# mikeferguson/ndt_2d

Hardware: AMD Instinct MI355X
Metric: pose-candidates x beams scored per second (higher is better)
Workload: dtype f64

## Files before the change

### ndt_2d_amd/csrc/ndt2d_device_fn.h

```cpp
#ifndef NDT2D_DEVICE_FN_H_
#define NDT2D_DEVICE_FN_H_

#include <hip/hip_runtime.h>
#include <math.h>

#include "ndt2d_kernels.h"

namespace ndt2d
{

constexpr int kWave = 64;
constexpr int kRecord = 12;
constexpr double kNoIndex = 1.0e308;
constexpr double kPadCoord = -1.0e300;

template <bool POW2>
__device__ __forceinline__ uint32_t cell_index(const GridDesc & g, double px, double py)
{
  const double tx = px - g.origin_x;
  const double ty = py - g.origin_y;
  double fx, fy;
  if (POW2)
  {
    fx = tx * g.inv_cell_size;
    fy = ty * g.inv_cell_size;
  }
  else
  {
    fx = tx / g.cell_size;
    fy = ty / g.cell_size;
  }
  const bool inside = (tx >= 0.0) & (ty >= 0.0) & (fx < static_cast<double>(g.size_x)) &
                      (fy < static_cast<double>(g.size_y));
  const uint32_t gx = static_cast<uint32_t>(fx);
  const uint32_t gy = static_cast<uint32_t>(fy);
  return inside ? gy * g.size_x + gx : g.ncell;
}

__device__ __forceinline__ double record_exponent(double mx, double my, double h00,
                                                  double h01, double h11, double px, double py)
{
  const double q0 = px - mx;
  const double q1 = py - my;
  const double r0 = q0 * h00 + q1 * h01;
  const double r1 = q0 * h01 + q1 * h11;
  return r0 * q0 + r1 * q1;
}

__device__ __forceinline__ double record_likelihood(double mx, double my, double h00,
                                                    double h01, double h11, double px,
                                                    double py)
{
  return exp(record_exponent(mx, my, h00, h01, h11, px, py));
}

__device__ __forceinline__ double fma3(double a, double b, double c)
{
  double d;
  asm("v_fma_f64 %0, %1, %2, %3" : "=v"(d) : "v"(a), "v"(b), "v"(c));
  return d;
}
#ifndef NDT2D_EXP_SCALAR_CONSTANTS
#define NDT2D_EXP_SCALAR_CONSTANTS 0
#endif
template <uint32_t HI, uint32_t LO>
__device__ __forceinline__ double fma3k(double a, double b)
{
  double d;
#if NDT2D_EXP_SCALAR_CONSTANTS
  uint32_t lo, hi;
  asm volatile("s_mov_b32 %0, %2\n\ts_mov_b32 %1, %3" : "=s"(lo), "=s"(hi) : "n"(LO), "n"(HI));
  const double c = __hiloint2double(static_cast<int>(hi), static_cast<int>(lo));
  asm("v_fma_f64 %0, %1, %2, %3" : "=v"(d) : "v"(a), "v"(b), "s"(c));
#else
  asm("v_fma_f64 %0, %1, %2, %3" : "=v"(d) : "v"(a), "v"(b), "v"(__hiloint2double(static_cast<int>(HI), static_cast<int>(LO))));
#endif
  return d;
}

__device__ __forceinline__ double exp_of_exponent(double x)
{
  asm("v_max_f64 %0, %1, %2" : "=v"(x) : "v"(x), "s"(-1000.0));
  const double n = rint(x * 1.4426950408889634);
  double r = fma(n, -0.6931471805599453, x);
  r = fma(n, -2.3190468138462996e-17, r);
  double p = fma3k<0x3e928af3u, 0xfca7ab0cu>(r, 0x1.ade156a5dcb37p-26);
  p = fma3k<0x3ec71deeu, 0x623fde64u>(r, p);
  p = fma3k<0x3efa0199u, 0x7c89e6b0u>(r, p);
  p = fma3k<0x3f2a01a0u, 0x14761f6eu>(r, p);
  p = fma3k<0x3f56c16cu, 0x1852b7b0u>(r, p);
  p = fma3k<0x3f811111u, 0x11122322u>(r, p);
  p = fma3k<0x3fa55555u, 0x555502a1u>(r, p);
  p = fma3k<0x3fc55555u, 0x55555511u>(r, p);
  p = fma3k<0x3fe00000u, 0x0000000bu>(r, p);
  asm("v_fma_f64 %0, %1, %2, 1.0" : "=v"(p) : "v"(r), "v"(p));
  asm("v_fma_f64 %0, %1, %2, 1.0" : "=v"(p) : "v"(r), "v"(p));
  return ldexp(p, static_cast<int>(n));
}

__device__ __forceinline__ bool wave_any(bool p)
{
  return __builtin_amdgcn_ballot_w64(p) != 0ull;
}

constexpr double kExpOverflowAbove = 0x1.62e42fefa39efp+9;

__device__ __forceinline__ double exp_score(double e)
{
  double r = exp_of_exponent(e);
  if (__builtin_expect(wave_any(!(e <= kExpOverflowAbove)), 0))
  {
    r = (e != e) ? e + e : (e > kExpOverflowAbove ? HUGE_VAL : r);
  }
  return r;
}

__device__ __forceinline__ double negligible_below(double s)
{
  const double from_sum =
    fma(static_cast<double>(__builtin_amdgcn_frexp_exp(s) - 1), 0.6931471805599453, -38.0);
  return (s > 0.0 && from_sum > -746.0) ? from_sum : -746.0;
}

template <bool LDS_GRID>
__device__ __forceinline__ double indexed_exponent(const GridDesc & g, const double * lds_cells,
                                                   uint32_t idx, double px, double py)
{
  double2 a, b, c;
  if (LDS_GRID)
  {
    const double2 * rec = reinterpret_cast<const double2 *>(lds_cells + idx * kCellDoubles);
    a = rec[0];
    b = rec[1];
    c = rec[2];
  }
  else
  {
    const double2 * rec =
      reinterpret_cast<const double2 *>(g.cells_global + static_cast<size_t>(idx) * kCellStrideGlobal);
    a = rec[0];
    b = rec[1];
    c = rec[2];
  }
  return record_exponent(a.x, a.y, b.x, b.y, c.x, px, py);
}

template <bool LDS_GRID>
__device__ __forceinline__ double indexed_likelihood(const GridDesc & g, const double * lds_cells,
                                                     uint32_t idx, double px, double py)
{
  return exp(indexed_exponent<LDS_GRID>(g, lds_cells, idx, px, py));
}

template <bool LDS_GRID, bool POW2>
__device__ __forceinline__ double point_likelihood(const GridDesc & g, const double * lds_cells,
                                                   double px, double py)
{
  return indexed_likelihood<LDS_GRID>(g, lds_cells, cell_index<POW2>(g, px, py), px, py);
}

__device__ __forceinline__ void stage_grid_to_lds(const GridDesc & g, double * lds_cells)
{
  const uint32_t n2 = (g.ncell + 1) * kCellDoubles / 2;
  const double2 * src = reinterpret_cast<const double2 *>(g.cells_lds_image);
  double2 * dst = reinterpret_cast<double2 *>(lds_cells);
  for (uint32_t i = threadIdx.x; i < n2; i += blockDim.x)
  {
    dst[i] = src[i];
  }
}

__device__ __forceinline__ double wave_sum(double v)
{
#pragma unroll
  for (int off = kWave / 2; off > 0; off >>= 1)
  {
    v += __shfl_xor(v, off, kWave);
  }
  return v;
}

constexpr int kDppQuadXor1 = 0xb1;
constexpr int kDppQuadXor2 = 0x4e;
constexpr int kDppRowHalfMirror = 0x141;
constexpr int kDppRowMirror = 0x140;
constexpr int kDppRowBcast15 = 0x142;
constexpr int kDppRowBcast31 = 0x143;

template <int CTRL, int ROW_MASK>
__device__ __forceinline__ double dpp_f64(double v, double fallback)
{
  const int lo = __builtin_amdgcn_update_dpp(__double2loint(fallback), __double2loint(v), CTRL,
                                             ROW_MASK, 0xf, false);
  const int hi = __builtin_amdgcn_update_dpp(__double2hiint(fallback), __double2hiint(v), CTRL,
                                             ROW_MASK, 0xf, false);
  return __hiloint2double(hi, lo);
}

__device__ __forceinline__ double wave_sum_to_last_lane(double v)
{
  v += dpp_f64<kDppQuadXor1, 0xf>(v, 0.0);
  v += dpp_f64<kDppQuadXor2, 0xf>(v, 0.0);
  v += dpp_f64<kDppRowHalfMirror, 0xf>(v, 0.0);
  v += dpp_f64<kDppRowMirror, 0xf>(v, 0.0);
  v += dpp_f64<kDppRowBcast15, 0xa>(v, 0.0);
  v += dpp_f64<kDppRowBcast31, 0xc>(v, 0.0);
  return v;
}

__device__ __forceinline__ double shortest_angular_distance(double from, double to)
{
  const double kPi = 3.14159265358979323846;
  const double r = fmod((to - from) + kPi, 2.0 * kPi);
  return r <= 0.0 ? r + kPi : r - kPi;
}

__device__ __forceinline__ void store_host(double * p, double v)
{
  __hip_atomic_store(p, v, __ATOMIC_RELAXED, __HIP_MEMORY_SCOPE_SYSTEM);
}
__device__ __forceinline__ void raise_host_flag(double * flag_slot, unsigned long long seq)
{
  asm volatile("s_waitcnt vmcnt(0)" ::: "memory");
  __hip_atomic_store(reinterpret_cast<unsigned long long *>(flag_slot), seq, __ATOMIC_RELAXED,
                     __HIP_MEMORY_SCOPE_SYSTEM);
}

#ifdef NDT2D_TEST_HOOKS
constexpr unsigned long long kDonePollTicks = 50ull * 1000 * 1000;
#else
constexpr unsigned long long kDonePollTicks = 1000ull * 1000 * 1000;
#endif
struct BoundedPoll
{
  uint32_t trips = 0;
  unsigned long long since = 0;
  __device__ __forceinline__ bool expired()
  {
    if ((++trips & 1023u) != 0u) return false;
    const unsigned long long now = wall_clock64();
    if (since == 0)
    {
      since = now | 1ull;
      return false;
    }
    return now - since > kDonePollTicks;
  }
};

#ifdef NDT2D_TEST_HOOKS
static __device__ int g_test_drop_done = 0;
#define NDT2D_TEST_DROPS_DONE(index) (g_test_drop_done != 0 && static_cast<uint32_t>(g_test_drop_done - 1) == static_cast<uint32_t>(index))
#else
#define NDT2D_TEST_DROPS_DONE(index) false
#endif

__device__ __forceinline__ bool better(double s_a, double i_a, double s_b, double i_b)
{
  return (s_a < s_b) | ((s_a == s_b) & (i_a < i_b));
}

constexpr int kNearTieLog2 = 36;

__device__ __forceinline__ void merge_best(double os, double oi, double & s, double & i)
{
  double larger;
  asm("v_max_f64 %0, |%1|, |%2|" : "=v"(larger) : "v"(os), "v"(s));
  const bool near = (ldexp(fabs(os - s), kNearTieLog2) <= larger) & (oi < kNoIndex) & (i < kNoIndex);
  if (better(os, oi, s, i))
  {
    s = os;
    i = oi;
  }
  if (near) i = floor(i) + 0.5;
}

template <int CTRL, int ROW_MASK>
__device__ __forceinline__ void best_step(double & s, double & i)
{
  const double os = dpp_f64<CTRL, ROW_MASK>(s, s);
  const double oi = dpp_f64<CTRL, ROW_MASK>(i, kNoIndex);
  merge_best(os, oi, s, i);
}

__device__ __forceinline__ void wave_best_to_last_lane(double & s, double & i)
{
  best_step<kDppQuadXor1, 0xf>(s, i);
  best_step<kDppQuadXor2, 0xf>(s, i);
  best_step<kDppRowHalfMirror, 0xf>(s, i);
  best_step<kDppRowMirror, 0xf>(s, i);
  best_step<kDppRowBcast15, 0xa>(s, i);
  best_step<kDppRowBcast31, 0xc>(s, i);
}

}

#endif
```

### ndt_2d_amd/csrc/ndt2d_match_lane.hip

```cpp
#include <cmath>
#include <cstdlib>

#include <type_traits>

#include "ndt2d_lane_fn.h"

namespace ndt2d
{

namespace
{

constexpr uint32_t kDynamicItemsFromBeams = 256;
constexpr int kLaneThreads = 1024;
constexpr int kLaneThreadsSmall = 256;
#ifndef NDT2D_LANE_THREADS_COMPACT
#define NDT2D_LANE_THREADS_COMPACT 768
#endif
constexpr int kLaneThreadsCompact = NDT2D_LANE_THREADS_COMPACT;
#define NDT2D_LANE_COMPACT_WAVES_PER_EU (NDT2D_LANE_THREADS_COMPACT / 128)

__global__ void __launch_bounds__(256) outer_table_kernel(const MatchArgs a, double4 * outer,
                                                          uint8_t * map_out, const LaneGeom geo)
{
  {
    const GridDesc & g = a.grid;
    const uint32_t n_map = static_cast<uint32_t>(kMapStride) * geo.map_h;
    for (uint32_t i = blockIdx.x * 256 + threadIdx.x; i < n_map; i += gridDim.x * 256)
    {
      const int32_t mx = static_cast<int32_t>(i & (kMapStride - 1));
      const int32_t my = static_cast<int32_t>(i >> 8);
      if (geo.block_log2 > 0)
      {
        const int32_t cells = 1 << geo.block_log2;
        map_out[i] = block_byte(g, mx * cells - geo.pad + geo.win_x0, my * cells - geo.pad + geo.win_y0, cells);
        continue;
      }
      const int32_t sub = 1 << geo.sub_log2;
      const int32_t cx = (mx >> geo.sub_log2) - geo.pad + geo.win_x0;
      const int32_t cy = (my >> geo.sub_log2) - geo.pad + geo.win_y0;
      map_out[i] = sub_cell_byte(g, cx, cy, mx & (sub - 1), my & (sub - 1), geo.sub_log2);
    }
  }

  if (blockIdx.x == 0 && threadIdx.x < kItemShards) a.next_item[threadIdx.x * kItemShardStride] = 0u;
  const uint64_t n = static_cast<uint64_t>(a.th_end - a.th_begin) * a.n_beams;
  for (uint64_t i = static_cast<uint64_t>(blockIdx.x) * 256 + threadIdx.x; i < n;
       i += static_cast<uint64_t>(gridDim.x) * 256)
  {
    const uint32_t t = static_cast<uint32_t>(i / a.n_beams);
    const uint32_t b = static_cast<uint32_t>(i - static_cast<uint64_t>(t) * a.n_beams);
    const uint32_t ith = a.th_begin + t * a.th_stride;
    const double ct = a.cos_th[ith];
    const double st = a.sin_th[ith];
    const double2 p = reinterpret_cast<const double2 *>(a.beams_xy)[b];
    double4 o;
    o.x = p.x * ct - p.y * st + a.pose_x;
    o.y = p.x * st + p.y * ct + a.pose_y;
    double kx = ((o.x - a.grid.origin_x) * a.grid.inv_cell_size + (geo.pad - geo.win_x0)) * geo.unit_scale;
    double ky = ((o.y - a.grid.origin_y) * a.grid.inv_cell_size + (geo.pad - geo.win_y0)) * geo.unit_scale;
    kx = !(kx >= geo.k_min) ? geo.k_min : (kx > geo.k_max_x ? geo.k_max_x : kx);
    ky = !(ky >= geo.k_min) ? geo.k_min : (ky > geo.k_max_y ? geo.k_max_y : ky);
    o.z = kTwo52 + (rint(ky) * kTwo24 + rint(kx)) + kNearBias;
    o.w = 0.0;
    outer[i] = o;
  }
}

__device__ __forceinline__ void item_step(uint32_t item, uint32_t patches, uint32_t th_mid, uint32_t & t,
                                          uint32_t & p)
{
  const uint32_t rank = item / patches;
  p = item - rank * patches;
  t = (rank & 1u) ? th_mid + (rank + 1u) / 2u : th_mid - rank / 2u;
}

__device__ __forceinline__ void item_place(uint32_t item, uint32_t patches, uint32_t patches_1d,
                                           uint32_t th_mid, uint32_t & t, uint32_t & pxi, uint32_t & pyi)
{
  uint32_t p;
  item_step(item, patches, th_mid, t, p);
  pxi = p / patches_1d;
  pyi = p - pxi * patches_1d;
}

__device__ __forceinline__ double packed_offset(double dx, double dy, double inv_scaled)
{
  return rint(dy * inv_scaled) * kTwo24 + rint(dx * inv_scaled);
}

__device__ __forceinline__ double no_index_here()
{
  static_assert(kNoIndex == 1.0e308, "the literal below is 1.0e308");
  uint32_t lo, hi;
  asm volatile("v_mov_b32 %0, 0x85ebc8a0\n\tv_mov_b32 %1, 0x7fe1ccf3" : "=v"(lo), "=v"(hi));
  return __hiloint2double(static_cast<int>(hi), static_cast<int>(lo));
}

template <int THREADS, bool POW2, bool LDS_RECORDS, bool DYNAMIC_ITEMS, bool COMPACT, bool PARTS = false,
          bool STRIPS = false>
__device__ __forceinline__ void match_lane_body(
  const MatchArgs & a, const double4 * __restrict__ outer, const uint8_t * __restrict__ map_image,
  const LaneGeom & geo)
{
  extern __shared__ __align__(16) double lds[];
  const GridDesc & g = a.grid;
#if defined(NDT2D_LANE_HIST) || defined(NDT2D_LANE_PATHS)
  if (blockIdx.x == 0 && threadIdx.x == 0) g_lane_hist = a.scores;
#endif
  uint8_t * lds_map = reinterpret_cast<uint8_t *>(lds);
  const uint32_t map_bytes = static_cast<uint32_t>(geo.map_h) * kMapStride;
  const uint32_t rank_bytes = COMPACT ? compact_rank_bytes(g.ncell) : 0u;
  double * lds_cells = lds + (map_bytes + rank_bytes) / sizeof(double);

  if (COMPACT)
  {
    const uint4 * src_rank = reinterpret_cast<const uint4 *>(g.cell_rank);
    uint4 * dst_rank = reinterpret_cast<uint4 *>(lds_map + map_bytes + kRankLead);
    for (uint32_t i = threadIdx.x; i < (rank_bytes - kRankLead) / 16; i += THREADS) dst_rank[i] = src_rank[i];
    if (threadIdx.x == 0)
    {
      reinterpret_cast<uint16_t *>(lds_map + map_bytes + kRankLead)[-1] = static_cast<uint16_t>(g.n_occ);
    }
    const uint32_t n2 = (g.n_occ + 1) * kCellDoubles / 2;
    const double2 * src = reinterpret_cast<const double2 *>(g.compact_records);
    double2 * dst = reinterpret_cast<double2 *>(lds_cells);
    for (uint32_t i = threadIdx.x; i < n2; i += THREADS) dst[i] = src[i];
  }
  else if (LDS_RECORDS)
  {
    stage_grid_to_lds(g, lds_cells);
  }
  {
    const uint32_t n16 = static_cast<uint32_t>(kMapStride) * geo.map_h / 16;
    const uint4 * src = reinterpret_cast<const uint4 *>(map_image);
    uint4 * dst = reinterpret_cast<uint4 *>(lds_map);
    for (uint32_t i = threadIdx.x; i < n16; i += THREADS) dst[i] = src[i];
  }
  __syncthreads();

#ifdef NDT2D_LANE_TRACE
  const unsigned long long trace_t0 = wall_clock64();
  unsigned long long trace_last = trace_t0, trace_max = 0, trace_last_start = trace_t0;
  uint32_t trace_items = 0, trace_prev_item = 0, trace_flagged = 0;
#endif
  LaneCtx c;
  c.rank_address = map_bytes + (COMPACT ? kRankLead : 0u);
  c.lds_cells_address = map_bytes + rank_bytes;
  c.sub_log2 = static_cast<uint32_t>(geo.sub_log2);
  c.exact_index = geo.block_log2 > 0 ? 1u : 0u;
  c.idx_bias = static_cast<uint32_t>(geo.pad - geo.win_y0) * g.size_x +
               static_cast<uint32_t>(geo.pad - geo.win_x0);
  c.size_x = g.size_x;

  const uint32_t lane = threadIdx.x & (kWave - 1);
  const uint32_t wave = __builtin_amdgcn_readfirstlane(threadIdx.x >> 6);
  const uint32_t n_lin = a.n_lin;
  static_assert(!STRIPS || (DYNAMIC_ITEMS && !PARTS), "strip tiles: the unsplit dynamic-item forms only");
  const LaneTiling tiling = lane_tiling(n_lin, STRIPS);
  const uint32_t patches = tiling.per_theta;
  const uint32_t n_items = (a.th_end - a.th_begin) * patches * (PARTS ? a.beam_parts : 1u);
  constexpr uint32_t kLaneWaves = THREADS / kWave;
  const uint32_t n_workers = gridDim.x * kLaneWaves;
  const uint32_t worker = wave * gridDim.x + blockIdx.x;
  const uint64_t per_theta = static_cast<uint64_t>(n_lin) * n_lin;
  const uint32_t th_mid = (a.th_end - a.th_begin - 1u) / 2u;
  const uint32_t home_shard = blockIdx.x % kItemShards;
  const double inv_scaled = geo.inv_scaled;

  double best_s = 0.0;
  double best_i = kNoIndex;
  double acc[10];
#pragma unroll
  for (int k = 0; k < 10; ++k) acc[k] = 0.0;
  for (uint32_t item = worker; item < n_items;)
  {
    uint32_t t, p;
#ifdef NDT2D_LANE_TRACE
    {
      const unsigned long long now = wall_clock64();
      if (trace_items > 0 && now - trace_last > trace_max) trace_max = now - trace_last;
      if (trace_items > 0 && a.scores != nullptr && lane == 0)
      {
        a.scores[5 * 8192 + 150000 + trace_prev_item] = static_cast<double>(now - trace_last);
        a.scores[5 * 8192 + 300000 + trace_prev_item] = static_cast<double>(trace_flagged);
      }
      trace_flagged = 0;
      trace_prev_item = item;
      trace_last = now;
      trace_last_start = now;
      ++trace_items;
      if (a.scores != nullptr && lane == 0) a.scores[5 * 8192 + item] = static_cast<double>(now);
    }
#endif
    const uint32_t whole_item = PARTS ? item / a.beam_parts : item;
    const uint32_t part = PARTS ? item - whole_item * a.beam_parts : 0u;
    item_step(whole_item, patches, th_mid, t, p);
    uint32_t x0, y0, h_log2, x_end;
    if (STRIPS)
    {
      lane_tile(tiling, n_lin, p, x0, y0, h_log2, x_end);
    }
    else
    {
      x0 = p / tiling.row * kPatch;
      y0 = (p - p / tiling.row * tiling.row) * kPatch;
      h_log2 = 3;
      x_end = n_lin;
    }
    const bool strip_tile = STRIPS && p >= tiling.core;
    uint32_t lane_here = lane;
    asm volatile("" : "+v"(lane_here));
    const uint32_t ix = x0 + (lane_here >> h_log2);
    const uint32_t iy = y0 + (lane_here & ((1u << h_log2) - 1u));
    const double dx = a.dlin[min(ix, x_end - 1)];
    const double dy = a.dlin[min(iy, n_lin - 1)];
    const double dxy = packed_offset(dx, dy, inv_scaled);
    const double4 * __restrict__ row = outer + static_cast<size_t>(t) * a.n_beams;

    double sum = 0.0;
    SkipState skip = skip_state(0.0, geo.no_skip);
    NDT2D_PATH(200, 1);
    const double dxy_corner = __hiloint2double(__builtin_amdgcn_readfirstlane(__double2hiint(dxy)),
                                               __builtin_amdgcn_readfirstlane(__double2loint(dxy)));
    const uint32_t beams_begin = PARTS ? part * a.part_beams : 0u;
    const uint32_t beams_end = PARTS ? min(beams_begin + a.part_beams, a.n_beams) : a.n_beams;
    for (uint32_t b0 = beams_begin; b0 < beams_end; b0 += kWave)
    {
      uint64_t can_score = ~0ull;
      if (geo.box_span >= 0)
      {
        const double k = row[min(b0 + lane, a.n_beams - 1u)].z;
        if (strip_tile)
        {
          const bool along_x = h_log2 < 3u;
          can_score = __builtin_amdgcn_ballot_w64(
            strip_can_score(k + dxy_corner, along_x ? geo.strip_span_long : geo.strip_span_short,
                            along_x ? geo.strip_span_short : geo.strip_span_long));
        }
        else
        {
          can_score = __builtin_amdgcn_ballot_w64(patch_can_score(k + dxy_corner, geo.box_span));
        }
        NDT2D_PATH(201, 1);
      }
#ifdef NDT2D_LANE_TRACE
      trace_flagged += static_cast<uint32_t>(__popcll(can_score));
#endif
      const uint32_t chunk_end = min(b0 + static_cast<uint32_t>(kWave), beams_end);
      uint32_t b = b0;
      for (; b + kUnroll <= chunk_end; b += kUnroll, can_score >>= kUnroll)
      {
        if ((can_score & ((1ull << kUnroll) - 1ull)) == 0ull) continue;
        double4 o[kUnroll];
#pragma unroll
        for (int u = 0; u < kUnroll; ++u) o[u] = row[b + u];
        __builtin_amdgcn_s_setprio(3);
        lane_beams<kUnroll, POW2, LDS_RECORDS, true, COMPACT>(g, c, o, dx, dy, dxy, sum, skip, geo.no_skip);
        __builtin_amdgcn_s_setprio(0);
      }
      for (; b < chunk_end; ++b, can_score >>= 1)
      {
        if ((can_score & 1ull) == 0ull) continue;
        const double4 one[1] = {row[b]};
        lane_beams<1, POW2, LDS_RECORDS, true, COMPACT>(g, c, one, dx, dy, dxy, sum, skip, geo.no_skip);
      }
    }

    if (PARTS)
    {
      a.part_sums[static_cast<size_t>(item) * kWave + lane] = sum;
      uint32_t next = n_items;
      if (lane == kWave - 1)
      {
        for (uint32_t tried = 0; tried < kItemShards && next >= n_items; ++tried)
        {
          const uint32_t shard = (home_shard + tried) % kItemShards;
          const uint32_t k = atomicAdd(a.next_item + shard * kItemShardStride, 1u);
          const uint64_t candidate = static_cast<uint64_t>(n_workers) + static_cast<uint64_t>(k) * kItemShards + shard;
          if (candidate < n_items) next = static_cast<uint32_t>(candidate);
        }
      }
      item = static_cast<uint32_t>(__builtin_amdgcn_readlane(static_cast<int>(next), kWave - 1));
      continue;
    }
    uint32_t lane_again = lane;
    asm volatile("" : "+v"(lane_again));
    const uint32_t ix_e = x0 + (lane_again >> h_log2);
    const uint32_t iy_e = y0 + (lane_again & ((1u << h_log2) - 1u));
    if ((ix_e < x_end) & (iy_e < n_lin))
    {
      const uint32_t ix = ix_e, iy = iy_e;
      const double score = -sum;
      const uint64_t local = static_cast<uint64_t>(t) * per_theta + static_cast<uint64_t>(ix) * n_lin + iy;
      const double flat = static_cast<double>(
        static_cast<uint64_t>(a.th_begin + t * a.th_stride) * per_theta + static_cast<uint64_t>(ix) * n_lin + iy);
      if (DYNAMIC_ITEMS)
      {
        if (score < best_s)
        {
          best_s = score;
          best_i = flat;
        }
      }
      else if (score < 0.0)
      {
        merge_best(score, flat, best_s, best_i);
      }
      const double dt = a.dth[a.th_begin + t * a.th_stride];
      acc[0] += (dx * dx) * score;
      acc[1] += (dx * dy) * score;
      acc[2] += (dx * dt) * score;
      acc[3] += (dy * dy) * score;
      acc[4] += (dy * dt) * score;
      acc[5] += (dt * dt) * score;
      acc[6] += dx * score;
      acc[7] += dy * score;
      acc[8] += dt * score;
      acc[9] += score;
#if !defined(NDT2D_LANE_HIST) && !defined(NDT2D_LANE_TRACE) && !defined(NDT2D_LANE_PATHS)
      if (a.scores != nullptr) a.scores[local] = score;
#endif
    }

    if (!DYNAMIC_ITEMS)
    {
      item += n_workers;
      continue;
    }
    if (wave_any(sum != 0.0))
    {
      NDT2D_PATH(209, 1);
      wave_best_to_last_lane(best_s, best_i);
#pragma unroll
      for (int k = 0; k < 10; ++k) acc[k] = wave_sum_to_last_lane(acc[k]);
    }

    uint32_t next = n_items;
    if (lane == kWave - 1)
    {
      double * out = a.partials + static_cast<size_t>(item) * kRecord;
      out[0] = best_s;
      out[1] = best_i;
#pragma unroll
      for (int k = 0; k < 10; ++k) out[2 + k] = acc[k];
      for (uint32_t tried = 0; tried < kItemShards && next >= n_items; ++tried)
      {
        const uint32_t shard = (home_shard + tried) % kItemShards;
        const uint32_t k = atomicAdd(a.next_item + shard * kItemShardStride, 1u);
        const uint64_t candidate = static_cast<uint64_t>(n_workers) + static_cast<uint64_t>(k) * kItemShards + shard;
        if (candidate < n_items) next = static_cast<uint32_t>(candidate);
      }
    }
    item = static_cast<uint32_t>(__builtin_amdgcn_readlane(static_cast<int>(next), kWave - 1));
    best_s = 0.0;
    best_i = no_index_here();
#pragma unroll
    for (int k = 0; k < 10; ++k) acc[k] = 0.0;
  }
#ifdef NDT2D_LANE_TRACE
  if (a.scores != nullptr && lane == 0)
  {
    const unsigned long long now = wall_clock64();
    if (trace_items > 0 && now - trace_last > trace_max) trace_max = now - trace_last;
    if (trace_items > 0) a.scores[5 * 8192 + 150000 + trace_prev_item] = static_cast<double>(now - trace_last);
    if (trace_items > 0) a.scores[5 * 8192 + 300000 + trace_prev_item] = static_cast<double>(trace_flagged);
    a.scores[5 * worker] = static_cast<double>(trace_t0);
    a.scores[5 * worker + 1] = static_cast<double>(now);
    a.scores[5 * worker + 2] = static_cast<double>(trace_items);
    a.scores[5 * worker + 3] = static_cast<double>(trace_max);
    a.scores[5 * worker + 4] = static_cast<double>(trace_last_start);
  }
#endif
  if (!DYNAMIC_ITEMS)
  {
    wave_best_to_last_lane(best_s, best_i);
#pragma unroll
    for (int k = 0; k < 10; ++k) acc[k] = wave_sum_to_last_lane(acc[k]);
    if (lane == kWave - 1)
    {
      double * out = a.partials + static_cast<size_t>(worker) * kRecord;
      out[0] = best_s;
      out[1] = best_i;
#pragma unroll
      for (int k = 0; k < 10; ++k) out[2 + k] = acc[k];
    }
  }
}

template <int THREADS, bool POW2, bool LDS_RECORDS, bool DYNAMIC_ITEMS, bool STRIPS = false>
__global__ void __launch_bounds__(THREADS) match_lane_kernel(
  const MatchArgs a, const double4 * __restrict__ outer, const uint8_t * __restrict__ map_image,
  const LaneGeom geo)
{
  match_lane_body<THREADS, POW2, LDS_RECORDS, DYNAMIC_ITEMS, false, false, STRIPS>(a, outer, map_image, geo);
}

template <bool STRIPS>
__global__ void __launch_bounds__(kLaneThreadsCompact) __attribute__((amdgpu_waves_per_eu(NDT2D_LANE_COMPACT_WAVES_PER_EU)))
match_lane_compact_kernel(const MatchArgs a, const double4 * __restrict__ outer,
                          const uint8_t * __restrict__ map_image, const LaneGeom geo)
{
  match_lane_body<kLaneThreadsCompact, true, true, true, true, false, STRIPS>(a, outer, map_image, geo);
}

template <bool POW2, bool STRIPS>
__global__ void __launch_bounds__(kLaneThreadsCompact) __attribute__((amdgpu_waves_per_eu(NDT2D_LANE_COMPACT_WAVES_PER_EU)))
match_lane_gather6_kernel(const MatchArgs a, const double4 * __restrict__ outer,
                          const uint8_t * __restrict__ map_image, const LaneGeom geo)
{
  match_lane_body<kLaneThreadsCompact, POW2, false, true, false, false, STRIPS>(a, outer, map_image, geo);
}

__global__ void __launch_bounds__(kLaneThreadsCompact) __attribute__((amdgpu_waves_per_eu(NDT2D_LANE_COMPACT_WAVES_PER_EU)))
match_lane_compact_parts_kernel(const MatchArgs a, const double4 * __restrict__ outer,
                                const uint8_t * __restrict__ map_image, const LaneGeom geo)
{
  match_lane_body<kLaneThreadsCompact, true, true, true, true, true>(a, outer, map_image, geo);
}

template <bool POW2>
__global__ void __launch_bounds__(kLaneThreadsCompact) __attribute__((amdgpu_waves_per_eu(NDT2D_LANE_COMPACT_WAVES_PER_EU)))
match_lane_gather6_parts_kernel(const MatchArgs a, const double4 * __restrict__ outer,
                                const uint8_t * __restrict__ map_image, const LaneGeom geo)
{
  match_lane_body<kLaneThreadsCompact, POW2, false, true, false, true>(a, outer, map_image, geo);
}

__global__ void __launch_bounds__(256) match_lane_combine_kernel(const MatchArgs a)
{
  const uint32_t lane = threadIdx.x & (kWave - 1);
  const uint32_t n_lin = a.n_lin;
  const uint32_t patches_1d = (n_lin + kPatch - 1) / kPatch;
  const uint32_t patches = patches_1d * patches_1d;
  const uint32_t n_items = (a.th_end - a.th_begin) * patches;
  const uint32_t item = blockIdx.x * 4u + (threadIdx.x >> 6);
  if (item >= n_items) return;
  const uint32_t th_mid = (a.th_end - a.th_begin - 1u) / 2u;
  uint32_t t, pxi, pyi;
  item_place(item, patches, patches_1d, th_mid, t, pxi, pyi);
  const uint32_t ix = pxi * kPatch + (lane >> 3);
  const uint32_t iy = pyi * kPatch + (lane & 7);
  const bool valid = (ix < n_lin) & (iy < n_lin);
  const double * p = a.part_sums + static_cast<size_t>(item) * a.beam_parts * kWave + lane;
  double sum = p[0];
  for (uint32_t j = 1; j < a.beam_parts; ++j) sum += p[static_cast<size_t>(j) * kWave];
  double best_s = 0.0;
  double best_i = kNoIndex;
  double acc[10];
#pragma unroll
  for (int k = 0; k < 10; ++k) acc[k] = 0.0;
  if (valid)
  {
    const double dx = a.dlin[ix];
    const double dy = a.dlin[iy];
    const double score = -sum;
    const uint64_t per_theta = static_cast<uint64_t>(n_lin) * n_lin;
    const uint64_t in_theta = static_cast<uint64_t>(ix) * n_lin + iy;
    const uint32_t ith = a.th_begin + t * a.th_stride;
    if (score < 0.0)
    {
      best_s = score;
      best_i = static_cast<double>(static_cast<uint64_t>(ith) * per_theta + in_theta);
    }
    const double dt = a.dth[ith];
    acc[0] = (dx * dx) * score;
    acc[1] = (dx * dy) * score;
    acc[2] = (dx * dt) * score;
    acc[3] = (dy * dy) * score;
    acc[4] = (dy * dt) * score;
    acc[5] = (dt * dt) * score;
    acc[6] = dx * score;
    acc[7] = dy * score;
    acc[8] = dt * score;
    acc[9] = score;
#ifndef NDT2D_LANE_TRACE
    if (a.scores != nullptr) a.scores[static_cast<uint64_t>(t) * per_theta + in_theta] = score;
#endif
  }
  wave_best_to_last_lane(best_s, best_i);
#pragma unroll
  for (int k = 0; k < 10; ++k) acc[k] = wave_sum_to_last_lane(acc[k]);
  if (lane == kWave - 1)
  {
    double * out = a.partials + static_cast<size_t>(item) * kRecord;
    out[0] = best_s;
    out[1] = best_i;
#pragma unroll
    for (int k = 0; k < 10; ++k) out[2 + k] = acc[k];
  }
}

bool pow2_grid(const MatchArgs & args) { return args.grid.pow2 != 0; }

uint32_t lane_beam_parts(const MatchArgs & args, uint32_t * part_beams)
{
  const uint64_t p1 = (args.n_lin + kPatch - 1) / kPatch;
  const uint64_t whole = static_cast<uint64_t>(args.n_th) * p1 * p1;
  uint32_t parts = whole < kPartsFourBelow ? 4u : (whole < kPartsTwoBelow ? 2u : 1u);
  if (const char * env = std::getenv("NDT2D_LANE_PARTS"))
  {
    const int v = std::atoi(env);
    if (v == 1 || v == 2 || v == 4 || v == 8) parts = static_cast<uint32_t>(v);
  }
  const uint32_t chunks = (args.n_beams + kWave - 1) / kWave;
  if (args.n_beams < kDynamicItemsFromBeams || parts > chunks) parts = 1;
  const uint32_t per_part = (chunks + parts - 1) / parts;
  *part_beams = per_part * kWave;
  return (chunks + per_part - 1) / per_part;
}

bool lane_records_in_lds(const MatchArgs & args, size_t map_bytes, size_t lds_per_block)
{
  const size_t grid_bytes = static_cast<size_t>(args.grid.ncell + 1) * kCellDoubles * sizeof(double);
  return grid_bytes + map_bytes <= lds_per_block;
}

}

bool lane_slabs(const MatchArgs & args, uint32_t * slab_th, uint32_t * n_slabs)
{
  const uint64_t p1 = (args.n_lin + kPatch - 1) / kPatch;
  const uint64_t per_theta = p1 * p1;
  const uint64_t th_total = args.th_end - args.th_begin;
  if (per_theta == 0 || th_total == 0 || per_theta > kMaxLaneItems) return false;
  uint64_t slab_items = kLaneSlabItems;
  if (const char * env = std::getenv("NDT2D_LANE_SLAB_ITEMS"))
  {
    const long long v = std::atoll(env);
    if (v > 0 && static_cast<uint64_t>(v) <= kMaxLaneItems) slab_items = static_cast<uint64_t>(v);
  }
  uint64_t th = slab_items / per_theta;
  if (th < 1) th = 1;
  const uint64_t at_least = (th_total + kMaxLaneSlabs - 1) / kMaxLaneSlabs;
  if (th < at_least) th = at_least;
  if (th > th_total) th = th_total;
  if (th * per_theta > kMaxLaneItems) return false;
  *slab_th = static_cast<uint32_t>(th);
  *n_slabs = static_cast<uint32_t>((th_total + th - 1) / th);
  return true;
}

size_t match_lane_outer_doubles(const MatchArgs & args)
{
  uint32_t slab_th = args.th_end - args.th_begin, n_slabs = 1;
  (void)lane_slabs(args, &slab_th, &n_slabs);
  uint32_t part_beams = 0;
  const uint32_t parts = lane_beam_parts(args, &part_beams);
  const uint64_t p1 = (args.n_lin + kPatch - 1) / kPatch;
  const size_t part_sums = parts > 1 ? static_cast<size_t>(slab_th) * p1 * p1 * parts * kWave : 0;
  return static_cast<size_t>(slab_th) * args.n_beams * 4 +
         static_cast<size_t>(kMapStride) * kMaxMapCells / sizeof(double) + part_sums;
}

bool match_lane_supported(const MatchArgs & args, size_t lds_per_block)
{
  LaneGeom geo;
  size_t map_bytes = 0;
  if (args.grid.occ_bits == nullptr || !lane_geometry(args, lds_per_block, &geo, &map_bytes)) return false;
  uint32_t slab_th = 0, n_slabs = 0;
  return map_bytes <= lds_per_block && lane_slabs(args, &slab_th, &n_slabs) &&
         args.grid.size_x < (1u << 24) && args.grid.ncell < (1u << 24);
}

hipError_t launch_match_lane(const MatchArgs & args_in, double * outer, double * workspace,
                             uint32_t max_workers, int cus, size_t lds_per_block, bool no_skip,
                             hipStream_t stream, hipEvent_t ev_after_pre_kernel,
                             uint32_t * n_workers_out, int * records_mode_out, uint32_t * parts_out)
{
  MatchArgs args = args_in;
  args.partials = workspace;
  LaneGeom geo;
  size_t map_bytes = 0;
  if (!lane_geometry(args, lds_per_block, &geo, &map_bytes)) return hipErrorInvalidValue;
  geo.no_skip = no_skip ? 1 : 0;
  {
    static const bool pretest = [] {
      const char * v = std::getenv("NDT2D_LANE_PRETEST");
      return v == nullptr || v[0] != '0';
    }();
    if (no_skip || !pretest) geo.box_span = -1;
  }
  const bool dynamic_items = args.n_beams >= kDynamicItemsFromBeams;
  const uint32_t p1 = (args.n_lin + kPatch - 1) / kPatch;
  const uint64_t n_items = static_cast<uint64_t>(args.th_end - args.th_begin) * p1 * p1;

  const uint64_t n_outer = static_cast<uint64_t>(args.th_end - args.th_begin) * args.n_beams;
  uint32_t oblocks = static_cast<uint32_t>((n_outer + 255) / 256);
  if (oblocks > 4096) oblocks = 4096;
  if (oblocks < 64) oblocks = 64;
  uint8_t * map_image = reinterpret_cast<uint8_t *>(outer + n_outer * 4);
  uint32_t part_beams = 0;
  uint32_t beam_parts = dynamic_items ? lane_beam_parts(args, &part_beams) : 1u;
  args.part_sums = outer + n_outer * 4 + static_cast<size_t>(kMapStride) * kMaxMapCells / sizeof(double);

  const char * knob_rec = std::getenv("NDT2D_LANE_RECORDS");
  const bool lds_records = lane_records_in_lds(args, map_bytes, lds_per_block) &&
                           !(knob_rec != nullptr && knob_rec[0] == 'g');
  size_t lds_bytes =
    map_bytes +
    (lds_records ? static_cast<size_t>(args.grid.ncell + 1) * kCellDoubles * sizeof(double) : 0);
  const size_t compact_bytes =
    compact_rank_bytes(args.grid.ncell) +
    (static_cast<size_t>(args.grid.n_occ) + 1) * kCellDoubles * sizeof(double);
  const char * knob = std::getenv("NDT2D_LANE_COMPACT");
  const bool compact_possible = dynamic_items && pow2_grid(args) && lds_records && args.grid.n_occ > 0 &&
                                args.grid.compact_records != nullptr &&
                                2 * (map_bytes + compact_bytes) <= lds_per_block &&
                                !(knob != nullptr && knob[0] == '0');
  const char * knob6 = std::getenv("NDT2D_LANE_GATHER6");
  const bool gather6_possible = dynamic_items && !lds_records && 2 * map_bytes <= lds_per_block &&
                                !(knob6 != nullptr && knob6[0] == '0');
  if (!(compact_possible || gather6_possible)) beam_parts = 1;
  args.beam_parts = beam_parts;
  args.part_beams = part_beams;
  if (!(dynamic_items && beam_parts == 1)) geo.strips = 0;
  const bool strips = geo.strips != 0;
  const uint64_t n_tiles =
    static_cast<uint64_t>(args.th_end - args.th_begin) * lane_tiling(args.n_lin, geo.strips != 0).per_theta;
  const uint64_t n_sub_items = beam_parts > 1 ? n_items * beam_parts : n_tiles;

  const bool small = beam_parts == 1 && n_items <= static_cast<uint64_t>(cus) * (kLaneThreadsSmall / kWave);
  const uint32_t waves_per_block = (small ? kLaneThreadsSmall : kLaneThreads) / kWave;
  uint32_t blocks = static_cast<uint32_t>((n_tiles + waves_per_block - 1) / waves_per_block);
  uint32_t max_blocks = static_cast<uint32_t>(cus);
  if (max_blocks * waves_per_block > max_workers) max_blocks = max_workers / waves_per_block;
  if (blocks > max_blocks) blocks = max_blocks;
  if (blocks == 0) blocks = 1;
  const bool compact = !small && compact_possible;
  const bool gather6 = !compact && !small && gather6_possible;
  if (records_mode_out != nullptr)
  {
    *records_mode_out = (compact ? 2 : (lds_records ? 1 : 0)) | (geo.block_log2 > 0 ? 4 : 0);
  }
  if (compact || gather6)
  {
    lds_bytes = compact ? map_bytes + compact_bytes : map_bytes;
    const uint32_t wpb = kLaneThreadsCompact / kWave;
    blocks = static_cast<uint32_t>((n_sub_items + wpb - 1) / wpb);
    uint32_t cap = 2 * static_cast<uint32_t>(cus);
    if (cap * wpb > max_workers) cap = max_workers / wpb;
    if (blocks > cap) blocks = cap;
    if (blocks == 0) blocks = 1;
  }
  hipLaunchKernelGGL(outer_table_kernel, dim3(oblocks), dim3(256), 0, stream, args,
                     reinterpret_cast<double4 *>(outer), map_image, geo);
  hipError_t e = hipGetLastError();
  if (e != hipSuccess) return e;
  if (ev_after_pre_kernel != nullptr)
  {
    e = hipEventRecord(ev_after_pre_kernel, stream);
    if (e != hipSuccess) return e;
  }
  auto launch = [&](auto kernel, int threads) -> hipError_t {
    const hipError_t e2 = prepare_absolute_lds_kernel(reinterpret_cast<const void *>(kernel), lds_bytes);
    if (e2 != hipSuccess) return e2;
    hipLaunchKernelGGL(kernel, dim3(blocks), dim3(threads), lds_bytes, stream, args,
                       reinterpret_cast<const double4 *>(outer),
                       static_cast<const uint8_t *>(map_image), geo);
    return hipGetLastError();
  };
  const bool pow2 = args.grid.pow2 != 0;
  auto pick = [&](auto threads_tag) -> hipError_t {
    constexpr int T = decltype(threads_tag)::value;
    auto with_items = [&](auto dyn_tag, auto strips_tag) -> hipError_t {
      constexpr bool D = decltype(dyn_tag)::value;
      constexpr bool S = decltype(strips_tag)::value;
      return lds_records ? (pow2 ? launch(match_lane_kernel<T, true, true, D, S>, T)
                                 : launch(match_lane_kernel<T, false, true, D, S>, T))
                         : (pow2 ? launch(match_lane_kernel<T, true, false, D, S>, T)
                                 : launch(match_lane_kernel<T, false, false, D, S>, T));
    };
    if (!dynamic_items) return with_items(std::false_type{}, std::false_type{});
    return strips ? with_items(std::true_type{}, std::true_type{}) : with_items(std::true_type{}, std::false_type{});
  };
  if (beam_parts > 1)
  {
    e = compact ? launch(match_lane_compact_parts_kernel, kLaneThreadsCompact)
                : (pow2 ? launch(match_lane_gather6_parts_kernel<true>, kLaneThreadsCompact)
                        : launch(match_lane_gather6_parts_kernel<false>, kLaneThreadsCompact));
    if (e == hipSuccess)
    {
      hipLaunchKernelGGL(match_lane_combine_kernel, dim3(static_cast<uint32_t>((n_items + 3) / 4)), dim3(256),
                         0, stream, args);
      e = hipGetLastError();
    }
  }
  else if (compact)
  {
    e = strips ? launch(match_lane_compact_kernel<true>, kLaneThreadsCompact)
               : launch(match_lane_compact_kernel<false>, kLaneThreadsCompact);
  }
  else if (gather6)
  {
    e = pow2 ? (strips ? launch(match_lane_gather6_kernel<true, true>, kLaneThreadsCompact)
                       : launch(match_lane_gather6_kernel<true, false>, kLaneThreadsCompact))
             : (strips ? launch(match_lane_gather6_kernel<false, true>, kLaneThreadsCompact)
                       : launch(match_lane_gather6_kernel<false, false>, kLaneThreadsCompact));
  }
  else
  {
    e = small ? pick(std::integral_constant<int, kLaneThreadsSmall>{})
              : pick(std::integral_constant<int, kLaneThreads>{});
  }
  if (parts_out != nullptr) *parts_out = beam_parts;
  if (n_workers_out != nullptr)
  {
    *n_workers_out = dynamic_items ? static_cast<uint32_t>(beam_parts > 1 ? n_items : n_tiles)
                                   : blocks * waves_per_block;
  }
  return e;
}

}
```

Before: 3083 billion.

## Use permlane swaps for wave reductions and 2D grid for outer table

Replaces the ten independent full-wave DPP reductions in the dynamic-item epilogue with a permlane32/permlane16 swap-add tree. This packs pairs of accumulators so fewer cross-lane ops are needed, and lanes 15/31/47/63 each write part of the record. Separately, the outer-table precompute kernel is launched on a 2D grid: rows for the map image, then one row per theta with beams along x. This removes the 64-bit division per element. It adds scattered stores from several lanes and relies on permlane swap builtins that only some targets provide.

```diff
diff --git a/ndt_2d_amd/csrc/ndt2d_device_fn.h b/ndt_2d_amd/csrc/ndt2d_device_fn.h
--- a/ndt_2d_amd/csrc/ndt2d_device_fn.h
+++ b/ndt_2d_amd/csrc/ndt2d_device_fn.h
@@ -208,6 +208,47 @@
   return v;
 }
 
+#ifndef NDT2D_LANE_SWAP_EPILOGUE
+#define NDT2D_LANE_SWAP_EPILOGUE 1
+#endif
+#if NDT2D_LANE_SWAP_EPILOGUE
+template <bool HALVES>
+__device__ __forceinline__ double swap_add(double a, double b)
+{
+  typedef unsigned int uint2v __attribute__((ext_vector_type(2)));
+  const unsigned int a_lo = static_cast<unsigned int>(__double2loint(a)), a_hi = static_cast<unsigned int>(__double2hiint(a));
+  const unsigned int b_lo = static_cast<unsigned int>(__double2loint(b)), b_hi = static_cast<unsigned int>(__double2hiint(b));
+  const uint2v lo = HALVES ? __builtin_amdgcn_permlane32_swap(a_lo, b_lo, false, false)
+                           : __builtin_amdgcn_permlane16_swap(a_lo, b_lo, false, false);
+  const uint2v hi = HALVES ? __builtin_amdgcn_permlane32_swap(a_hi, b_hi, false, false)
+                           : __builtin_amdgcn_permlane16_swap(a_hi, b_hi, false, false);
+  return __hiloint2double(static_cast<int>(hi[0]), static_cast<int>(lo[0])) +
+         __hiloint2double(static_cast<int>(hi[1]), static_cast<int>(lo[1]));
+}
+
+__device__ __forceinline__ double row_sum_to_every_lane(double v)
+{
+  v += dpp_f64<kDppQuadXor1, 0xf>(v, 0.0);
+  v += dpp_f64<kDppQuadXor2, 0xf>(v, 0.0);
+  v += dpp_f64<kDppRowHalfMirror, 0xf>(v, 0.0);
+  v += dpp_f64<kDppRowMirror, 0xf>(v, 0.0);
+  return v;
+}
+
+__device__ __forceinline__ void wave_ten_sums_to_rows(const double (&acc)[10], double & r0, double & r1, double & r2)
+{
+  double p[5];
+#pragma unroll
+  for (int j = 0; j < 5; ++j) p[j] = swap_add<true>(acc[2 * j], acc[2 * j + 1]);
+  r0 = row_sum_to_every_lane(swap_add<false>(p[0], p[1]));
+  r1 = row_sum_to_every_lane(swap_add<false>(p[2], p[3]));
+  r2 = row_sum_to_every_lane(p[4]);
+  r2 += dpp_f64<kDppRowBcast15, 0xa>(r2, 0.0);
+}
+
+__device__ __forceinline__ uint32_t swap_sum_of_row(uint32_t w) { return ((w & 1u) << 1) | (w >> 1); }
+#endif
+
 __device__ __forceinline__ double shortest_angular_distance(double from, double to)
 {
   const double kPi = 3.14159265358979323846;
diff --git a/ndt_2d_amd/csrc/ndt2d_match_lane.hip b/ndt_2d_amd/csrc/ndt2d_match_lane.hip
--- a/ndt_2d_amd/csrc/ndt2d_match_lane.hip
+++ b/ndt_2d_amd/csrc/ndt2d_match_lane.hip
@@ -20,13 +20,32 @@
 constexpr int kLaneThreadsCompact = NDT2D_LANE_THREADS_COMPACT;
 #define NDT2D_LANE_COMPACT_WAVES_PER_EU (NDT2D_LANE_THREADS_COMPACT / 128)
 
+#ifndef NDT2D_LANE_TABLE_2D
+#define NDT2D_LANE_TABLE_2D 1
+#endif
+constexpr uint32_t kTableMaxRows = 65535;
+
 __global__ void __launch_bounds__(256) outer_table_kernel(const MatchArgs a, double4 * outer,
-                                                          uint8_t * map_out, const LaneGeom geo)
-{
+                                                          uint8_t * map_out, const LaneGeom geo
+#if NDT2D_LANE_TABLE_2D
+                                                          , const uint32_t map_rows
+#endif
+                                                          )
+{
+#if NDT2D_LANE_TABLE_2D
+  if (blockIdx.y < map_rows)
+#endif
   {
     const GridDesc & g = a.grid;
     const uint32_t n_map = static_cast<uint32_t>(kMapStride) * geo.map_h;
-    for (uint32_t i = blockIdx.x * 256 + threadIdx.x; i < n_map; i += gridDim.x * 256)
+#if NDT2D_LANE_TABLE_2D
+    const uint32_t map_first = (blockIdx.y * gridDim.x + blockIdx.x) * 256 + threadIdx.x;
+    const uint32_t map_step = map_rows * gridDim.x * 256;
+#else
+    const uint32_t map_first = blockIdx.x * 256 + threadIdx.x;
+    const uint32_t map_step = gridDim.x * 256;
+#endif
+    for (uint32_t i = map_first; i < n_map; i += map_step)
     {
       const int32_t mx = static_cast<int32_t>(i & (kMapStride - 1));
       const int32_t my = static_cast<int32_t>(i >> 8);
@@ -43,6 +62,15 @@
     }
   }
 
+#if NDT2D_LANE_TABLE_2D
+  if (blockIdx.x == 0 && blockIdx.y == 0 && threadIdx.x < kItemShards) a.next_item[threadIdx.x * kItemShardStride] = 0u;
+  if (blockIdx.y < map_rows) return;
+  const uint32_t b = blockIdx.x * 256 + threadIdx.x;
+  if (b >= a.n_beams) return;
+  for (uint32_t t = blockIdx.y - map_rows; t < a.th_end - a.th_begin; t += gridDim.y - map_rows)
+  {
+    const uint64_t i = static_cast<uint64_t>(t) * a.n_beams + b;
+#else
   if (blockIdx.x == 0 && threadIdx.x < kItemShards) a.next_item[threadIdx.x * kItemShardStride] = 0u;
   const uint64_t n = static_cast<uint64_t>(a.th_end - a.th_begin) * a.n_beams;
   for (uint64_t i = static_cast<uint64_t>(blockIdx.x) * 256 + threadIdx.x; i < n;
@@ -50,6 +78,7 @@
   {
     const uint32_t t = static_cast<uint32_t>(i / a.n_beams);
     const uint32_t b = static_cast<uint32_t>(i - static_cast<uint64_t>(t) * a.n_beams);
+#endif
     const uint32_t ith = a.th_begin + t * a.th_stride;
     const double ct = a.cos_th[ith];
     const double st = a.sin_th[ith];
@@ -288,6 +317,9 @@
     asm volatile("" : "+v"(lane_again));
     const uint32_t ix_e = x0 + (lane_again >> h_log2);
     const uint32_t iy_e = y0 + (lane_again & ((1u << h_log2) - 1u));
+#if NDT2D_LANE_SWAP_EPILOGUE
+    if (DYNAMIC_ITEMS) best_i = no_index_here();
+#endif
     if ((ix_e < x_end) & (iy_e < n_lin))
     {
       const uint32_t ix = ix_e, iy = iy_e;
@@ -328,6 +360,25 @@
       item += n_workers;
       continue;
     }
+#if NDT2D_LANE_SWAP_EPILOGUE
+    double sums_a = acc[0], sums_b = acc[4], sums_c = acc[8];
+    if (wave_any(sum != 0.0))
+    {
+      NDT2D_PATH(209, 1);
+      wave_ten_sums_to_rows(acc, sums_a, sums_b, sums_c);
+      wave_best_to_last_lane(best_s, best_i);
+    }
+    uint32_t lane_out = lane;
+    asm volatile("" : "+v"(lane_out));
+    if ((lane_out & 15u) == 15u)
+    {
+      const uint32_t w = lane_out >> 4;
+      double * out = a.partials + static_cast<size_t>(item) * kRecord + 2;
+      out[swap_sum_of_row(w)] = sums_a;
+      out[4u + swap_sum_of_row(w)] = sums_b;
+      if ((w & 1u) != 0u) out[8u + (w >> 1)] = sums_c;
+    }
+#else
     if (wave_any(sum != 0.0))
     {
       NDT2D_PATH(209, 1);
@@ -335,6 +386,7 @@
 #pragma unroll
       for (int k = 0; k < 10; ++k) acc[k] = wave_sum_to_last_lane(acc[k]);
     }
+#endif
 
     uint32_t next = n_items;
     if (lane == kWave - 1)
@@ -342,8 +394,10 @@
       double * out = a.partials + static_cast<size_t>(item) * kRecord;
       out[0] = best_s;
       out[1] = best_i;
+#if !NDT2D_LANE_SWAP_EPILOGUE
 #pragma unroll
       for (int k = 0; k < 10; ++k) out[2 + k] = acc[k];
+#endif
       for (uint32_t tried = 0; tried < kItemShards && next >= n_items; ++tried)
       {
         const uint32_t shard = (home_shard + tried) % kItemShards;
@@ -354,7 +408,9 @@
     }
     item = static_cast<uint32_t>(__builtin_amdgcn_readlane(static_cast<int>(next), kWave - 1));
     best_s = 0.0;
+#if !NDT2D_LANE_SWAP_EPILOGUE
     best_i = no_index_here();
+#endif
 #pragma unroll
     for (int k = 0; k < 10; ++k) acc[k] = 0.0;
   }
@@ -586,9 +642,11 @@
   const uint64_t n_items = static_cast<uint64_t>(args.th_end - args.th_begin) * p1 * p1;
 
   const uint64_t n_outer = static_cast<uint64_t>(args.th_end - args.th_begin) * args.n_beams;
+#if !NDT2D_LANE_TABLE_2D
   uint32_t oblocks = static_cast<uint32_t>((n_outer + 255) / 256);
   if (oblocks > 4096) oblocks = 4096;
   if (oblocks < 64) oblocks = 64;
+#endif
   uint8_t * map_image = reinterpret_cast<uint8_t *>(outer + n_outer * 4);
   uint32_t part_beams = 0;
   uint32_t beam_parts = dynamic_items ? lane_beam_parts(args, &part_beams) : 1u;
@@ -643,8 +701,22 @@
     if (blocks > cap) blocks = cap;
     if (blocks == 0) blocks = 1;
   }
+#if NDT2D_LANE_TABLE_2D
+  {
+    const uint32_t beam_blocks = (args.n_beams + 255u) / 256u;
+    const uint32_t map_blocks = static_cast<uint32_t>(map_bytes + 255) / 256u;
+    uint32_t th_rows = args.th_end - args.th_begin;
+    if (beam_blocks == 0 || th_rows == 0) return hipErrorInvalidValue;
+    const uint32_t map_rows = (map_blocks + beam_blocks - 1u) / beam_blocks;
+    if (map_rows >= kTableMaxRows) return hipErrorInvalidValue;
+    if (th_rows > kTableMaxRows - map_rows) th_rows = kTableMaxRows - map_rows;
+    hipLaunchKernelGGL(outer_table_kernel, dim3(beam_blocks, map_rows + th_rows), dim3(256), 0, stream, args,
+                       reinterpret_cast<double4 *>(outer), map_image, geo, map_rows);
+  }
+#else
   hipLaunchKernelGGL(outer_table_kernel, dim3(oblocks), dim3(256), 0, stream, args,
                      reinterpret_cast<double4 *>(outer), map_image, geo);
+#endif
   hipError_t e = hipGetLastError();
   if (e != hipSuccess) return e;
   if (ev_after_pre_kernel != nullptr)
```

New measurement: 3123 billion, median of 6. 1.01x the previous value.
